# DuckTapeDevOps/kubernetes-cloud

Measured on AMD Instinct MI355X. Metric: GPT-J-6B finetune tokens/sec, higher is better.
Workload: dtype bf16; 1 GPU; model=gpt-j-6b, global_batch=32, micro_batch=16, grad_accum=2, seq_len=2048, parallelism=dp1, activation_checkpointing=False

## Files before the change

csrc/kernels/attention.hip:

```cpp
#include "common.h"

#define LOG2E 1.4426950408889634f
#define LN2 0.6931471805599453f

struct AttnParams {
  const bf16_t* q; const bf16_t* k; const bf16_t* v;
  bf16_t* o; float* lse;
  long long q_sb, q_st, q_sh, k_sb, k_st, k_sh, v_sb, v_st, v_sh;
  long long o_sb, o_st, o_sh;
  int B, Sq, Sk, H, Hkv, d_real, causal;
  float scale;
  const float* alibi;
  const int* kv_len;
  const int* fix_flags;
  int window;
  const unsigned* key_mask;
  int km_words;
};

struct AttnBwdParams {
  const bf16_t* q; const bf16_t* k; const bf16_t* v; const bf16_t* o;
  const bf16_t* dout; bf16_t* dq; bf16_t* dk; bf16_t* dv;
  const float* lse; const float* delta;
  long long q_sb, q_st, q_sh, k_sb, k_st, k_sh, v_sb, v_st, v_sh;
// ... 822 lines not shown
                                    long long do_sh, int B, int S, int H,
                                    int d_real, hipStream_t stream) {
  int nc = (d_real + 7) / 8;
  int tpr = 1;
  while (tpr < nc && tpr < 64) tpr <<= 1;
  const int rpb = 256 / tpr;
  const long long rows = (long long)B * H * S;
  const long long grid = (rows + rpb - 1) / rpb;
  hipLaunchKernelGGL(attn_bwd_preprocess_kernel, dim3((unsigned)grid), dim3(256), 0, stream,
                     (const bf16_t*)o, (const bf16_t*)dout, delta, o_sb, o_st, o_sh,
                     do_sb, do_st, do_sh, B, S, H, d_real, tpr);
  return 0;
}

KCA_API int kca_attn_bwd_tiled(const void* q, const void* k, const void* v, const void* dout,
                               void* dq, void* dk, void* dv, const float* lse, const float* delta,
                               long long q_sb, long long q_st, long long q_sh, long long k_sb,
                               long long k_st, long long k_sh, long long v_sb, long long v_st,
                               long long v_sh, long long do_sb, long long do_st, long long do_sh,
                               long long dq_sb, long long dq_st, long long dq_sh, long long dk_sb,
                               long long dk_st, long long dk_sh, long long dv_sb, long long dv_st,
                               long long dv_sh, int B, int Sq, int Sk, int H, int Hkv, int d,
                               int causal, float scale, hipStream_t stream);

KCA_API int kca_attn_bwd(const void* q, const void* k, const void* v,
                         const void* o, const void* dout, void* dq, void* dk,
                         void* dv, const float* lse, const float* delta,
                         long long q_sb, long long q_st, long long q_sh,
                         long long k_sb, long long k_st, long long k_sh,
                         long long v_sb, long long v_st, long long v_sh,
                         long long do_sb, long long do_st, long long do_sh,
                         long long dq_sb, long long dq_st, long long dq_sh,
                         long long dk_sb, long long dk_st, long long dk_sh,
                         long long dv_sb, long long dv_st, long long dv_sh,
                         int B, int Sq, int Sk, int H, int Hkv, int d_real,
                         int causal, float scale, const float* alibi,
                         const int* kv_len, int window, const unsigned* key_mask, hipStream_t stream) {
  if (d_real % 8 || H % Hkv || window < 0) return 1;
  if (g_attn_tiled && !alibi && !kv_len && !window && !key_mask &&
      kca_attn_bwd_tiled(q, k, v, dout, dq, dk, dv, lse, delta, q_sb, q_st, q_sh, k_sb, k_st, k_sh,
                         v_sb, v_st, v_sh, do_sb, do_st, do_sh, dq_sb, dq_st, dq_sh, dk_sb, dk_st,
                         dk_sh, dv_sb, dv_st, dv_sh, B, Sq, Sk, H, Hkv, d_real, causal, scale,
                         stream) == 0)
    return 0;
  const int D = pick_d(d_real);
  AttnBwdParams p{(const bf16_t*)q, (const bf16_t*)k, (const bf16_t*)v, (const bf16_t*)o,
                  (const bf16_t*)dout, (bf16_t*)dq, (bf16_t*)dk, (bf16_t*)dv, lse, delta,
                  q_sb, q_st, q_sh, k_sb, k_st, k_sh, v_sb, v_st, v_sh,
                  do_sb, do_st, do_sh, dq_sb, dq_st, dq_sh, dk_sb, dk_st, dk_sh,
                  dv_sb, dv_st, dv_sh,
                  B, Sq, Sk, H, Hkv, d_real, causal, scale, alibi, kv_len, window, key_mask, (Sk + 31) / 32};
  if (D == 256) {
    dim3 h2(((Sq + 127) / 128) * B * H);
    dim3 g1w(((Sk + 63) / 64) * B * Hkv);
    if (causal) {
      hipLaunchKernelGGL((attn_bwd_dkdv_kernel<256, true>), g1w, dim3(256), 0, stream, p);
      hipLaunchKernelGGL((attn_bwd_dq32_kernel<256, true>), h2, dim3(256), 0, stream, p);
    } else {
      hipLaunchKernelGGL((attn_bwd_dkdv_kernel<256, false>), g1w, dim3(256), 0, stream, p);
      hipLaunchKernelGGL((attn_bwd_dq32_kernel<256, false>), h2, dim3(256), 0, stream, p);
    }
    return 0;
  }
  dim3 g1(((Sk + 63) / 64) * B * Hkv);
  dim3 g2(((Sq + 63) / 64) * B * H);
  ATTN_D_DISPATCH(D, {
    if (causal) {
      hipLaunchKernelGGL((attn_bwd_dkdv_kernel<DD, true>), g1, dim3(256), 0, stream, p);
      hipLaunchKernelGGL((attn_bwd_dq_kernel<DD, true>), g2, dim3(256), 0, stream, p);
    } else {
      hipLaunchKernelGGL((attn_bwd_dkdv_kernel<DD, false>), g1, dim3(256), 0, stream, p);
      hipLaunchKernelGGL((attn_bwd_dq_kernel<DD, false>), g2, dim3(256), 0, stream, p);
    }
  });
  return 0;
}
```

csrc/kernels/attention_tiled.hip:

```cpp
#include "common.h"

#include <type_traits>

namespace {

constexpr float kLog2e = 1.4426950408889634f;
constexpr float kLn2 = 0.6931471805599453f;
constexpr float kRescaleThr = 8.0f;

#ifdef KCA_ATTN_STAMPS
__device__ unsigned long long g_attn_stamps[64];
__device__ __forceinline__ unsigned long long ast_now() {
  unsigned long long t;
  __builtin_amdgcn_sched_barrier(0);
  asm volatile("s_memtime %0\n\ts_waitcnt lgkmcnt(0)" : "=s"(t)::"memory");
  __builtin_amdgcn_sched_barrier(0);
  return t;
}
#define ASTAMP_DECL                                            \
  unsigned long long st_acc_[8] = {0, 0, 0, 0, 0, 0, 0, 0}; \
  unsigned long long st_prev_ = ast_now();
#define ASTAMP(k)                           \
  do {                                      \
    const unsigned long long n_ = ast_now(); \
// ... 669 lines not shown
    const int lid128 = bh * nqb128 + (CAUSAL ? nqb128 - 1 - qb128 : qb128);
    if (lane == 0) p.flags[lid128 * 4 + w128] = any_bad;
  }
  const float inv = ltot > 0.f ? 1.f / ltot : 0.f;
  if (hh == 0 && p.lse)
    p.lse[((long long)b * p.H + h) * p.Sq + qrow] = ltot > 0.f ? (m + log2f(ltot)) * kLn2 : INFINITY;
  asm volatile("s_waitcnt vmcnt(0) lgkmcnt(0)" ::: "memory");
  __syncthreads();
  store_tile_lds<D, D>(p.o + b * p.o_sb + h * p.o_sh + (long long)q0 * p.o_st, p.o_st, oacc, lane, inv,
                       smem + wave * 32 * D * 2);
  ASTAMP(6);
  ASTAMP_FLUSH(48);
}

struct FastBwdParams {
  const bf16_t* q; const bf16_t* k; const bf16_t* v; const bf16_t* dout;
  bf16_t* dq; bf16_t* dk; bf16_t* dv;
  const float* lse; const float* delta;
  long long q_sb, q_st, q_sh, k_sb, k_st, k_sh, v_sb, v_st, v_sh, do_sb, do_st, do_sh;
  long long dq_sb, dq_st, dq_sh, dk_sb, dk_st, dk_sh, dv_sb, dv_st, dv_sh;
  int B, Sq, Sk, H, Hkv;
  float scale;
};

template <int D>
__device__ __forceinline__ void row_bases(int l32, int hh, int& e, int& o) {
  const int xr = (l32 >> 2) & 3;
  e = (l32 >> 3) * 16 * D + 64 * (l32 & 7) + 16 * (hh ^ xr);
  o = (l32 >> 3) * 16 * D + 64 * (l32 & 7) + 16 * ((2 + hh) ^ xr);
}
template <int D>
__device__ __forceinline__ void tr_bases(int lane, int& b1, int& b2) {
  const int hh = lane >> 5, gi = lane & 15;
  const int c3 = 2 * ((lane >> 4) & 1) + ((gi & 3) >> 1);
  b1 = 64 * (4 * hh + (gi >> 2)) + 16 * (c3 ^ hh) + 8 * (gi & 1);
  b2 = 16 * D + 64 * (4 * hh + (gi >> 2)) + 16 * (c3 ^ hh ^ 2) + 8 * (gi & 1);
}
template <int D>
__device__ __forceinline__ bf16x8 tr_frag(const char* img, int b1, int b2, int s, int db) {
  return cat8(lds_tr4(img, b1 + 2 * s * 16 * D + 512 * db), lds_tr4(img, b2 + 2 * s * 16 * D + 512 * db));
}
template <int D>
__device__ __forceinline__ bf16x8 row_frag(const char* img, int be, int bo, int s) {
  return lds_b128(img, ((s & 1) ? bo : be) + 512 * (s >> 1));
}

// ... 130 lines not shown
        if (db + 1 < D / 32) {
          t0[(db + 1) & 1] = tr_frag<D>(Ks, b1, b2, 0, db + 1);
          t1[(db + 1) & 1] = tr_frag<D>(Ks, b1, b2, 1, db + 1);
          __builtin_amdgcn_sched_group_barrier(0x100, 4, 0);
        }
        dq[db] = __builtin_amdgcn_mfma_f32_32x32x16_bf16(t0[db & 1], d0, dq[db], 0, 0, 0);
        dq[db] = __builtin_amdgcn_mfma_f32_32x32x16_bf16(t1[db & 1], d1, dq[db], 0, 0, 0);
        __builtin_amdgcn_sched_group_barrier(0x8, 2, 0);
      }
    }
    ASTAMP(4);
    asm volatile("" ::: "memory");
    if (t + 1 < ntiles) stg.store(sk, sv, smem + ((t + 1) & 1) * 2 * TILE);
    __syncthreads();
    ASTAMP(5);
  };
  const int nfree = CAUSAL ? ntiles - 4 : ntiles;
  for (int t = 0; t < nfree; ++t) tile_step(t, std::false_type{});
  for (int t = max(nfree, 0); t < ntiles; ++t) tile_step(t, std::true_type{});
  store_tile_lds<D, DS>(p.dq + b * p.dq_sb + h * p.dq_sh + (long long)q0 * p.dq_st, p.dq_st, dq, lane, p.scale,
                        smem + wave * 32 * D * 2);
  ASTAMP(6);
  ASTAMP_FLUSH(16);
}

template <int D, bool CAUSAL, int DS = D>
__global__ void __launch_bounds__(256, (D <= 64 && !CAUSAL) ? 3 : 1) attn_bwd_dkdv_tiled_kernel(FastBwdParams p) {
  constexpr int BK = 128, BQ = 32;
  constexpr int TILE = BQ * D * 2;
  using Stg = StagerFor<D, DS>;
  constexpr int NCH = D / 8, NCS = DS / 8, CPT = Stg::CPT;
  constexpr int KSD = DS / 16;
  constexpr int VOFF = 4 * TILE;
  constexpr int LOFF = VOFF + 4 * TILE;
  __shared__ __attribute__((aligned(16))) char smem[LOFF + 2 * 64 * 4];
  ASTAMP_DECL

  const int tid = threadIdx.x, lane = tid & 63, wave = tid >> 6;
  const int l32 = lane & 31, hh = lane >> 5;
  const int nkb = p.Sk / BK;
  const int lid = xcd_remap(blockIdx.x, gridDim.x);
  const int kb = lid % nkb, bh = lid / nkb;
  const int b = bh / p.Hkv, hk = bh % p.Hkv;
  const int grp = p.H / p.Hkv;
  const int off = p.Sk - p.Sq;
  const int kw = kb * BK + wave * 32;
// ... 149 lines not shown
    }
    ASTAMP(4);
    asm volatile("" ::: "memory");
    if (it + 1 < total) KCA_DKDV_STORE((it + 1) & 1);
    __syncthreads();
    ASTAMP(5);
  };
  for (int it = 0; it < total; ++it) tile_step(it, std::integral_constant<bool, CAUSAL>{});
#undef KCA_DKDV_LOAD
#undef KCA_DKDV_STORE
  if constexpr (D == 96) {
    store_acc_t<D>(p.dk + b * p.dk_sb + hk * p.dk_sh + (long long)key * p.dk_st, dk, hh, p.scale);
    store_acc_t<D>(p.dv + b * p.dv_sb + hk * p.dv_sh + (long long)key * p.dv_st, dv, hh, 1.f);
  } else {
    store_tile_lds<D, DS>(p.dk + b * p.dk_sb + hk * p.dk_sh + (long long)kw * p.dk_st, p.dk_st, dk, lane, p.scale,
                      smem + wave * 32 * D * 2);
    store_tile_lds<D, DS>(p.dv + b * p.dv_sb + hk * p.dv_sh + (long long)kw * p.dv_st, p.dv_st, dv, lane, 1.f,
                      smem + wave * 32 * D * 2);
  }
  ASTAMP(6);
  ASTAMP_FLUSH(32);
}

template <int D, bool CAUSAL>
__global__ void __launch_bounds__(512, 1) attn_bwd_dkdv_w8_kernel(FastBwdParams p) {
  constexpr int BK = 128, BQ = 32;
  constexpr int TILE = BQ * D * 2;
  using Stg = Stager<D, true, 512>;
  constexpr int CPT = Stg::CPT, KSD = D / 16;
  constexpr int PSZ = 4 * 64 * 16;
  constexpr int POFF = 3 * 2 * TILE;
  constexpr int LOFF = POFF + 2 * 4 * PSZ;
  __shared__ __attribute__((aligned(16))) char smem[LOFF + 3 * 64 * 4];
  static_assert(8 * 32 * D * 2 <= LOFF, "epilogue images of the 8 waves");
  ASTAMP_DECL

  const int tid = threadIdx.x, lane = tid & 63;
  const int wave = __builtin_amdgcn_readfirstlane(tid >> 6);
  const int pw = wave & 3;
  const bool kside = wave < 4;
  const int l32 = lane & 31, hh = lane >> 5;
  const int nkb = p.Sk / BK;
  const int lid = xcd_remap(blockIdx.x, gridDim.x);
  const int kb = lid % nkb, bh = lid / nkb;
  const int b = bh / p.H, h = bh % p.H;
  const int off = p.Sk - p.Sq;
  const int kw = kb * BK + pw * 32;
  const int key = kw + l32;
// ... 105 lines not shown
        for (int i = 0; i < D / 16; ++i) {
          if (i + 2 < D / 16) {
            f[(i + 2) % 3] = tr_frag<D>(Gs, b1, b2, i & 1, (i + 2) >> 1);
            __builtin_amdgcn_sched_group_barrier(0x100, 2, 0);
          }
          acc[i >> 1] = __builtin_amdgcn_mfma_f32_32x32x16_bf16(f[i % 3], (i & 1) ? p1 : p0, acc[i >> 1], 0, 0, 0);
          __builtin_amdgcn_sched_group_barrier(0x8, 1, 0);
        }
      }
      ASTAMP(4);
      asm volatile("" ::: "memory");
      if (t + 1 < total) store_tile(nxt);
      __syncthreads();
      ASTAMP(5);
    };
    int cur = 0;
    for (int t = 0; t < total; ++t) {
      const int nxt = cur == 2 ? 0 : cur + 1;
      v_step(t, cur, nxt);
      cur = nxt;
    }
    __syncthreads();
  } else {
    auto k_step = [&](int t, int cur, int nxt) {
      const char* Qs = smem + cur * 2 * TILE;
      const char* Gs = Qs + TILE;
      const float* ls = reinterpret_cast<const float*>(smem + LOFF) + cur * 64 + 32;
      const float* pb = reinterpret_cast<const float*>(smem + POFF + ((t & 1) * 4 + pw) * PSZ);
      ASTAMP(1);
      f32x16 dpacc;
#pragma unroll
      for (int r = 0; r < 16; ++r) dpacc[r] = 0.f;
      {
        constexpr int PF = 1;
        bf16x8 f[PF + 1];
#pragma unroll
        for (int s = 0; s < PF; ++s) f[s] = row_frag<D>(Gs, be, bo, s);
        __builtin_amdgcn_sched_group_barrier(0x100, PF, 0);
#pragma unroll
        for (int s = 0; s < KSD; ++s) {
          if (s + PF < KSD) {
            f[(s + PF) % (PF + 1)] = row_frag<D>(Gs, be, bo, s + PF);
            __builtin_amdgcn_sched_group_barrier(0x100, 1, 0);
          }
          dpacc = __builtin_amdgcn_mfma_f32_32x32x16_bf16(f[s % (PF + 1)], rf[s], dpacc, 0, 0, 0);
          __builtin_amdgcn_sched_group_barrier(0x8, 1, 0);
        }
      }
      ASTAMP(2);
      load_tile(min(t + 2, total - 1));
      asm volatile("" ::: "memory");
      bf16x8 s0, s1;
#pragma unroll
      for (int g = 0; g < 4; ++g) {
        const f32x4 pg = *reinterpret_cast<const f32x4*>(pb + (g * 64 + lane) * 4);
        const f32x4 dq4 = *reinterpret_cast<const f32x4*>(ls + 8 * g + 4 * hh);
#pragma unroll
        for (int j = 0; j < 4; ++j) {
          const int r = 4 * g + j;
          const float ds = pg[j] * (dpacc[r] - dq4[j]);
          if (r < 8) s0[r] = (__bf16)ds;
          else s1[r - 8] = (__bf16)ds;
        }
      }
      ASTAMP(3);
      {
        bf16x8 f[3];
        f[0] = tr_frag<D>(Qs, b1, b2, 0, 0);
        f[1] = tr_frag<D>(Qs, b1, b2, 1, 0);
        __builtin_amdgcn_sched_group_barrier(0x100, 4, 0);
#pragma unroll
        for (int i = 0; i < D / 16; ++i) {
          if (i + 2 < D / 16) {
            f[(i + 2) % 3] = tr_frag<D>(Qs, b1, b2, i & 1, (i + 2) >> 1);
            __builtin_amdgcn_sched_group_barrier(0x100, 2, 0);
          }
          acc[i >> 1] = __builtin_amdgcn_mfma_f32_32x32x16_bf16(f[i % 3], (i & 1) ? s1 : s0, acc[i >> 1], 0, 0, 0);
          __builtin_amdgcn_sched_group_barrier(0x8, 1, 0);
        }
      }
      ASTAMP(4);
      asm volatile("" ::: "memory");
      if (t + 2 < total) store_tile(nxt);
      __syncthreads();
      ASTAMP(5);
    };
    if (total > 1) {
// ... 6 lines not shown
      const int nxt = cur == 0 ? 2 : cur - 1;
      k_step(t, cur, nxt);
      cur = cur == 2 ? 0 : cur + 1;
    }
  }
  __builtin_amdgcn_s_setprio(0);
  {
    bf16_t* dst = kside ? p.dk + b * p.dk_sb + h * p.dk_sh + (long long)kw * p.dk_st
                        : p.dv + b * p.dv_sb + h * p.dv_sh + (long long)kw * p.dv_st;
    store_tile_lds<D>(dst, kside ? p.dk_st : p.dv_st, acc, lane, kside ? p.scale : 1.f, smem + wave * 32 * D * 2);
  }
  ASTAMP(6);
  if (!kside) {
    ASTAMP_FLUSH(40);
  } else {
    ASTAMP_FLUSH(56);
  }
}

inline bool offsets_fit(long long rows, long long stride) { return (rows + 128) * stride * 2 < (1ll << 31); }

}

static int g_attn_variant = 3;
KCA_API int kca_attn_set_variant(int v) {
  g_attn_variant = v;
  return 0;
}

KCA_API int kca_attn_fwd_tiled(const void* q, const void* k, const void* v, void* o, float* lse,
                               long long q_sb, long long q_st, long long q_sh, long long k_sb,
                               long long k_st, long long k_sh, long long v_sb, long long v_st,
                               long long v_sh, long long o_sb, long long o_st, long long o_sh,
                               int B, int Sq, int Sk, int H, int Hkv, int d, int causal,
                               float scale, int rowsum_col, int max_col, int* flags, hipStream_t stream) {
  if ((d != 48 && d != 64 && d != 96 && d != 128 && d != 160 && d != 256) || Sq % 128 || Sk % 32 || Sq <= 0 ||
      H % Hkv || !flags)
    return 1;
  if (max_col >= 0 && (max_col != 40 || rowsum_col != 40 || d != 48)) return 1;
  if (d == 48 && causal) return 1;
  if (rowsum_col >= 0 && (rowsum_col != 40 || (d != 64 && d != 48) || causal)) return 1;
  if (causal && Sk < Sq) return 1;
  if (!offsets_fit(Sk, k_st) || !offsets_fit(Sk, v_st)) return 1;
  FastFwdParams p{(const bf16_t*)q, (const bf16_t*)k, (const bf16_t*)v, (bf16_t*)o, lse, flags,
                  q_sb, q_st, q_sh, k_sb, k_st, k_sh, v_sb, v_st, v_sh, o_sb, o_st, o_sh,
                  B, Sq, Sk, H, Hkv, scale};
  dim3 grid((Sq / 128) * B * H);
// ... 93 lines not shown
      hipLaunchKernelGGL((attn_bwd_dkdv_tiled_kernel<96, false>), g1, dim3(256), 0, stream, p);
      hipLaunchKernelGGL((attn_bwd_dq_tiled_kernel<96, false>), g2, dim3(256), 0, stream, p);
    }
  } else if (d == 128) {
    if (causal) {
      hipLaunchKernelGGL((attn_bwd_dkdv_tiled_kernel<128, true>), g1, dim3(256), 0, stream, p);
      hipLaunchKernelGGL((attn_bwd_dq_tiled_kernel<128, true>), g2, dim3(256), 0, stream, p);
    } else {
      hipLaunchKernelGGL((attn_bwd_dkdv_tiled_kernel<128, false>), g1, dim3(256), 0, stream, p);
      hipLaunchKernelGGL((attn_bwd_dq_tiled_kernel<128, false>), g2, dim3(256), 0, stream, p);
    }
  } else {
    if (causal) {
      hipLaunchKernelGGL((attn_bwd_dkdv_tiled_kernel<64, true>), g1, dim3(256), 0, stream, p);
      hipLaunchKernelGGL((attn_bwd_dq_tiled_kernel<64, true>), g2, dim3(256), 0, stream, p);
    } else {
      hipLaunchKernelGGL((attn_bwd_dkdv_tiled_kernel<64, false>), g1, dim3(256), 0, stream, p);
      hipLaunchKernelGGL((attn_bwd_dq_tiled_kernel<64, false>), g2, dim3(256), 0, stream, p);
    }
  }
  return 0;
}

#ifdef KCA_ATTN_STAMPS
KCA_API int kca_attn_stamps(unsigned long long* host, int reset) {
  if (hipMemcpyFromSymbol(host, HIP_SYMBOL(g_attn_stamps), sizeof(unsigned long long) * 64) != hipSuccess) return 1;
  if (reset) {
    unsigned long long z[64] = {0};
    if (hipMemcpyToSymbol(HIP_SYMBOL(g_attn_stamps), z, sizeof(z)) != hipSuccess) return 1;
  }
  return 0;
}
#endif
```

kubernetes_cloud_amd/ops/_lib.py:

```python
from __future__ import annotations

import ctypes
import os
import threading

import torch

_HERE = os.path.dirname(os.path.abspath(__file__))
LIB_DIR = os.path.join(os.path.dirname(_HERE), "_lib")
DEBUG = os.environ.get("KCA_DEBUG", "0") in ("1", "true")
KERNEL_LIB = os.path.join(LIB_DIR, "libkca_kernels_debug.so" if DEBUG else "libkca_kernels.so")
KERNEL_LIB = os.environ.get("KCA_KERNEL_LIB") or KERNEL_LIB
ATTN_VARIANT_ENV = os.environ.get("KCA_ATTN_VARIANT")

_lock = threading.Lock()
_lib = None
_err: str | None = None

P = ctypes.c_void_p
I = ctypes.c_int
LL = ctypes.c_longlong
F = ctypes.c_float

_SIGS = {
# ... 7 lines not shown
    "kca_gelu_bwd": [P, P, P, LL, I, P],
    "kca_quick_gelu_fwd": [P, P, LL, P],
    "kca_quick_gelu_bwd": [P, P, P, LL, P],
    "kca_geglu_fwd": [P, P, LL, I, P],
    "kca_add_bias_nhwc": [P, P, P, P, LL, I, P],
    "kca_add_bias2_nhwc": [P, P, P, P, P, LL, I, P],
    "kca_colsum_bf16": [P, P, I, I, I, P],
    "kca_geglu_bwd": [P, P, P, LL, I, P],
    "kca_rope": [P, P, I, I, LL, I, LL, LL, LL, LL, I, I, P, P, P, F, P],
    "kca_accum_grad": [P, P, F, I, LL, P],
    "kca_accum_grad_pair": [P, P, P, F, LL, P],
    "kca_accum_grad_multi": [P, I, F, P],
    "kca_cast_f32_bf16": [P, P, LL, P],
    "kca_ema": [P, P, F, LL, P],
    "kca_cross_entropy_fwd": [P, LL, P, I, I, I, P, P, P],
    "kca_cross_entropy_bwd": [P, LL, P, P, P, F, I, I, I, P, LL, P],
    "kca_adamw": [P, P, P, P, P, LL, P, F, F, F, F, F, F, F, P, P, P],
    "kca_sumsq": [P, LL, P, P, P],
    "kca_adamw8bit": [P, P, P, P, P, P, P, LL, P, F, F, F, F, F, F, F, P, P, P],
    "kca_clip_coef": [P, F, F, P, P, P, P],
    "kca_attn_fwd": [P] * 5 + [LL] * 12 + [I] * 7 + [F, P, P, I, P, I, I, P, P],
    "kca_attn_bwd_preprocess": [P, P, P, LL, LL, LL, LL, LL, LL, I, I, I, I, P],
    "kca_attn_bwd": [P] * 10 + [LL] * 21 + [I] * 7 + [F, P, P, I, P, P],
    "kca_attn_fwd_wide": [P] * 5 + [LL] * 12 + [I] * 6 + [F, P, P],
    "kca_attn_set_tiled": [I],
    "kca_attn_set_variant": [I],
    "kca_transpose_bf16": [P, LL, P, LL, I, I, P],
    "kca_gelu_fwd_t": [P, LL, P, LL, P, LL, I, I, I, P],
    "kca_gelu_bwd_t": [P, LL, P, LL, P, LL, P, LL, P, I, I, I, P],
    "kca_transpose_colsum": [P, LL, P, LL, P, I, I, P],
    "kca_col_reduce_f32": [P, I, I, P, P, P],
    "kca_accum_grad_2d": [P, P, LL, I, I, F, I, P],
    "kca_groupnorm_fwd": [P, P, P, P, P, P, P, I, I, I, I, F, I, P],
    "kca_groupnorm_bwd": [P, P, P, P, P, P, P, P, P, P, I, I, I, I, I, P],
    "kca_groupnorm_nhwc_ws": [I, I, I],
    "kca_groupnorm_nhwc_fwd": [P, P, P, P, P, P, P, I, I, I, I, F, I, P],
    "kca_groupnorm_nhwc_fwd_add": [P, P, P, P, LL, P, P, P, P, I, I, I, I, F, I, P],
    "kca_groupnorm_nhwc_cat_fwd": [P, P, P, P, P, P, P, P, P, P, I, I, I, I, I, I, F, I, P],
    "kca_groupnorm_nhwc_bwd": [P, P, P, P, P, P, P, P, P, P, I, I, I, I, I, P],
    "kca_skinny_set_smallk": [I],
    "kca_conv3x3_fwd": [P, P, P, P, I, I, I, I, I, P],
    "kca_conv3x3_set_variant": [I],
    "kca_conv3x3_wflip": [P, P, I, I, P],
    "kca_conv3x3_wgrad_splits": [I, I, I, I, I],
    "kca_conv3x3_wgrad": [P, P, P, P, I, I, I, I, I, I, P],
    "kca_skinny_gemm": [P, LL, P, P, P, LL, I, I, I, I, P],
# ... 3 lines not shown
    "kca_ln_rows": [P, LL, P, P, P, LL, P, P, F, P, I, I, P],
    "kca_embed_ln_rows": [P, LL, P, P, P, I, P, LL, P, P, F, P, I, I, P],
    "kca_decode_prep": [P, LL, I, I, I, I, I, I, P, P, P, P, P, P, LL, LL, LL, P, I, I, P],
    "kca_decode_chunk": [I, I, I],
    "kca_decode_set_stamps": [P],
    "kca_decode_attn": [P, LL, P, P, LL, LL, LL, P, P, P, LL, P, LL, I, I, I, I, I, I, F, P, P, I, I, I, P],
    "kca_sd_noise_prep": [P, P, P, P, P, P, P, P, P, I, I, I, I, F, I, ctypes.c_ulonglong, LL, I, P],
    "kca_mse_split_fwd": [P, P, LL, LL, F, P, I, P, P],
    "kca_mse_split_bwd": [P, P, P, LL, LL, F, P, P],
    "kca_sd_lms_step": [P, P, P, P, LL, P, I, I, I, I, I, F, F, F, P],
    "kca_decode_prep_attn": [P, LL, P, P, LL, LL, LL, P, P, P, LL, P, LL, I, I, I, I, I, I, F, P, P, I, I, I, I, P,
                             P, I, I, P],
    "kca_im2col2x2_nhwc": [P, P, I, I, I, I, P],
    "kca_phase_to_dense_nhwc": [P, P, P, I, I, I, I, P],
    "kca_upsample2x_nhwc": [P, P, I, I, I, I, P],
    "kca_dense_to_phase_nhwc": [P, P, I, I, I, I, P],
    "kca_col2im2x2_nhwc": [P, P, I, I, I, I, P],
    "kca_pad_br_nhwc": [P, P, I, I, I, I, P],
    "kca_gemv_dual_ln": [P, P, I, P, P, I, P, P, P, P, P, P, P, F, P, P, P, P, I, P],
    "kca_sample_logits": [P, LL, I, I, I, P, P, P, P, P, P, P, I, P, LL, P, P, P, P, P, I, P],
}


_SIGS["kca_decode_prep_attn_gemv"] = _SIGS["kca_decode_prep_attn"][:-2] + [P, P, P, P, I, I, I, I, P]

for _n in ("kca_decode_prep_attn", "kca_ln_rows", "kca_embed_ln_rows", "kca_decode_prep_attn_gemv",
           "kca_gemv_dual_ln", "kca_skinny_gemm"):
    _SIGS[_n + "_f16"] = _SIGS[_n]


def _load():
    global _lib, _err
    if _lib is not None or _err is not None:
        return _lib
    with _lock:
        if _lib is not None or _err is not None:
            return _lib
        if not os.path.exists(KERNEL_LIB):
            _err = f"{KERNEL_LIB} not built (run `python tools/build_ext.py`)"
            return None
        try:
            lib = ctypes.CDLL(KERNEL_LIB, mode=ctypes.RTLD_GLOBAL)
        except OSError as e:
            _err = f"failed to load {KERNEL_LIB}: {e}"
            return None
        for name, argtypes in _SIGS.items():
            fn = getattr(lib, name, None)
            if fn is None:
                continue
            fn.argtypes = argtypes
            fn.restype = ctypes.c_int
        if ATTN_VARIANT_ENV is not None and hasattr(lib, "kca_attn_set_variant"):
            lib.kca_attn_set_variant(int(ATTN_VARIANT_ENV))
        _lib = lib
        return _lib


def available() -> bool:
    return _load() is not None


def require():
    lib = _load()
    if lib is None:
        raise RuntimeError(
            "kubernetes_cloud_amd native kernels unavailable: " + str(_err)
            + " -- refusing to fall back to eager PyTorch on a GPU tensor")
    return lib


def has(name: str) -> bool:
    lib = _load()
    return lib is not None and hasattr(lib, name)

# ... 57 lines not shown
```

kubernetes_cloud_amd/ops/attention.py:

```python
from __future__ import annotations

import math

import torch

from . import _lib
from .rope import apply_rotary_


def attention_reference(q, k, v, causal: bool, scale: float | None = None,
                        kv_len: torch.Tensor | None = None, alibi: torch.Tensor | None = None,
                        window: int = 0):
    B, Sq, H, D = q.shape
    Sk, Hkv = k.shape[1], k.shape[2]
    scale = scale if scale is not None else 1.0 / math.sqrt(D)
    qf = q.float().transpose(1, 2)
    kf = k.float().transpose(1, 2)
    vf = v.float().transpose(1, 2)
    if Hkv != H:
        rep = H // Hkv
        kf = kf.repeat_interleave(rep, dim=1)
        vf = vf.repeat_interleave(rep, dim=1)
    s = torch.matmul(qf, kf.transpose(-1, -2)) * scale
    qi = torch.arange(Sq, device=q.device)[:, None]
# ... 2 lines not shown
    if alibi is not None:
        s = s + alibi.float().view(1, H, 1, 1) * (ki - qi - off).float()
    mask = torch.zeros(B, 1, Sq, Sk, dtype=torch.bool, device=q.device)
    if causal:
        mask = mask | (ki > qi + off)
    if window:
        mask = mask | (ki <= qi + off - window)
    if kv_len is not None and kv_len.dtype == torch.bool:
        mask = mask | ~kv_len.to(q.device).view(B, 1, 1, Sk)
    elif kv_len is not None:
        mask = mask | (ki[None, None] >= kv_len.view(B, 1, 1, 1).to(q.device))
    s = s.masked_fill(mask, float("-inf"))
    lse = torch.logsumexp(s, dim=-1)
    p = torch.exp(s - lse[..., None])
    p = torch.nan_to_num(p, nan=0.0)
    o = torch.matmul(p, vf).transpose(1, 2)
    return o.to(q.dtype), lse


def set_tiled_path(enable: bool) -> None:
    _lib.call("kca_attn_set_tiled", int(bool(enable)))


DEFAULT_VARIANT = 3
_VARIANT = [int(_lib.ATTN_VARIANT_ENV) if _lib.ATTN_VARIANT_ENV is not None else DEFAULT_VARIANT]


def set_variant(v: int) -> int:
    _lib.call("kca_attn_set_variant", int(v))
    old, _VARIANT[0] = _VARIANT[0], int(v)
    return old


def _strides(t):
    return t.stride(0), t.stride(1), t.stride(2)


def pack_key_mask(mask: torch.Tensor) -> torch.Tensor:
    B, Sk = mask.shape
    W = (Sk + 31) // 32
    m = torch.zeros(B, W * 32, dtype=torch.int64, device=mask.device)
    m[:, :Sk] = mask.to(torch.int64)
    words = (m.view(B, W, 32) << torch.arange(32, device=mask.device, dtype=torch.int64)).sum(-1)
    words = torch.where(words >= 2 ** 31, words - 2 ** 32, words)
    return words.to(torch.int32).contiguous()


def _masks(kv_len):
    if kv_len is None:
        return None, None
    return (kv_len, None) if kv_len.dim() == 1 else (None, kv_len)


def _fwd(q, k, v, causal, scale, kv_len, alibi, out=None, window: int = 0, rowsum_col: int = -1,
         max_col: int = -1, lse=None, flags=None):
    B, Sq, H, D = q.shape
    Sk, Hkv = k.shape[1], k.shape[2]
    o = out if out is not None else torch.empty(B, Sq, H, D, device=q.device, dtype=q.dtype)
    if lse is None:
        lse = torch.empty(B, H, Sq, device=q.device, dtype=torch.float32)
    if flags is None:
        flags = torch.empty(4 * ((Sq + 127) // 128) * B * H, device=q.device, dtype=torch.int32)
    lens, km = _masks(kv_len)
    _lib.call("kca_attn_fwd", q.data_ptr(), k.data_ptr(), v.data_ptr(), o.data_ptr(), lse.data_ptr(),
              *_strides(q), *_strides(k), *_strides(v), *_strides(o),
              B, Sq, Sk, H, Hkv, D, int(causal), float(scale), _lib.ptr(alibi), _lib.ptr(lens),
              int(window), _lib.ptr(km), int(rowsum_col), int(max_col), flags.data_ptr(), _lib.stream())
    return o, lse


def _bwd(q, k, v, o, do, lse, dq, dk, dv, causal, scale, kv_len, alibi, window: int = 0):
    B, Sq, H, D = q.shape
    Sk, Hkv = k.shape[1], k.shape[2]
    delta = torch.empty(B, H, Sq, device=q.device, dtype=torch.float32)
    _lib.call("kca_attn_bwd_preprocess", o.data_ptr(), do.data_ptr(), delta.data_ptr(),
              *_strides(o), *_strides(do), B, Sq, H, D, _lib.stream())
    _lib.call("kca_attn_bwd", q.data_ptr(), k.data_ptr(), v.data_ptr(), o.data_ptr(), do.data_ptr(),
              dq.data_ptr(), dk.data_ptr(), dv.data_ptr(), lse.data_ptr(), delta.data_ptr(),
              *_strides(q), *_strides(k), *_strides(v), *_strides(do),
              *_strides(dq), *_strides(dk), *_strides(dv),
              B, Sq, Sk, H, Hkv, D, int(causal), float(scale), _lib.ptr(alibi), _lib.ptr(_masks(kv_len)[0]),
              int(window), _lib.ptr(_masks(kv_len)[1]), _lib.stream())


def _check(q, k, v):
    for t in (q, k, v):
        if t.dim() != 4 or t.stride(-1) != 1:
            raise ValueError("attention expects [B, S, H, D] views with unit last stride")
        if t.dtype != torch.bfloat16:
            raise ValueError("native attention is bf16")
    D = q.shape[-1]
    if D % 8 or D > 256:
        raise ValueError(f"head_dim {D} unsupported (multiple of 8, <= 256)")


class _FlashAttnFn(torch.autograd.Function):
    @staticmethod
    def forward(ctx, q, k, v, causal, scale, kv_len, alibi, window):
        _check(q, k, v)
        o, lse = _fwd(q, k, v, causal, scale, kv_len, alibi, window=window)
        ctx.save_for_backward(q, k, v, o, lse, kv_len, alibi)
        ctx.causal, ctx.scale, ctx.window = causal, scale, window
        return o

    @staticmethod
    def backward(ctx, do):
        q, k, v, o, lse, kv_len, alibi = ctx.saved_tensors
        do = do.contiguous()
        dq = torch.empty(q.shape, device=q.device, dtype=q.dtype)
        dk = torch.empty(k.shape, device=k.device, dtype=k.dtype)
        dv = torch.empty(v.shape, device=v.device, dtype=v.dtype)
        _bwd(q, k, v, o, do, lse, dq, dk, dv, ctx.causal, ctx.scale, kv_len, alibi, ctx.window)
        return dq, dk, dv, None, None, None, None, None


def native_mask(kv_len, device):
    if kv_len is None:
        return None
    if kv_len.dtype == torch.bool:
        return pack_key_mask(kv_len.to(device))
    return kv_len.to(device=device, dtype=torch.int32).contiguous()


def flash_attention(q: torch.Tensor, k: torch.Tensor, v: torch.Tensor, causal: bool = False,
                    scale: float | None = None, kv_len: torch.Tensor | None = None,
                    alibi: torch.Tensor | None = None, window: int = 0, rowsum_col: int = -1,
                    max_col: int = -1) -> torch.Tensor:
    scale = scale if scale is not None else 1.0 / math.sqrt(q.shape[-1])
    if alibi is not None:
        alibi = alibi.to(device=q.device, dtype=torch.float32).contiguous()
    if rowsum_col >= 0 and _lib.use_native(q, k, v) and not torch.is_grad_enabled():
        _check(q, k, v)
        return _fwd(q, k, v, causal, scale, native_mask(kv_len, q.device), alibi, window=window,
                    rowsum_col=rowsum_col, max_col=max_col)[0]
    if max_col >= 0:
# ... 29 lines not shown
    @staticmethod
    def forward(ctx, qkv, H, D, rot, interleaved, base, causal, scale, kv_len):
        B, S, _ = qkv.shape
        v5 = qkv.view(B, S, 3, H, D)
        q, k, v = v5[:, :, 0], v5[:, :, 1], v5[:, :, 2]
        if rot > 0:
            apply_rotary_(q, k, rot, S, interleaved, base, 1.0)
        o, lse = _fwd(q, k, v, causal, scale, kv_len, None)
        ctx.save_for_backward(qkv, o, lse, kv_len)
        ctx.cfg = (H, D, rot, interleaved, base, causal, scale)
        return o.view(B, S, H * D)

    @staticmethod
    def backward(ctx, do):
        qkv, o, lse, kv_len = ctx.saved_tensors
        H, D, rot, interleaved, base, causal, scale = ctx.cfg
        B, S, _ = qkv.shape
        v5 = qkv.view(B, S, 3, H, D)
        q, k, v = v5[:, :, 0], v5[:, :, 1], v5[:, :, 2]
        dqkv = torch.empty_like(qkv)
        d5 = dqkv.view(B, S, 3, H, D)
        dq, dk, dv = d5[:, :, 0], d5[:, :, 1], d5[:, :, 2]
        do = do.contiguous().view(B, S, H, D)
        _bwd(q, k, v, o, do, lse, dq, dk, dv, causal, scale, kv_len, None)
        if rot > 0:
            apply_rotary_(dq, dk, rot, S, interleaved, base, -1.0)
        return dqkv, None, None, None, None, None, None, None, None


def qkv_rope_attention(qkv: torch.Tensor, n_heads: int, head_dim: int, rot: int,
                       interleaved: bool, causal: bool = True, base: float = 10000.0,
                       scale: float | None = None,
                       kv_len: torch.Tensor | None = None) -> torch.Tensor:
    B, S, _ = qkv.shape
    scale = scale if scale is not None else 1.0 / math.sqrt(head_dim)
    if _lib.use_native(qkv):
        return _QKVRopeAttnFn.apply(qkv.contiguous(), n_heads, head_dim, rot, interleaved, base,
                                    causal, scale, native_mask(kv_len, qkv.device))
    v5 = qkv.view(B, S, 3, n_heads, head_dim)
    q, k, v = v5[:, :, 0], v5[:, :, 1], v5[:, :, 2]
    if rot > 0:
        q, k = _rope_out_of_place(q, k, rot, interleaved, base)
    o, _ = attention_reference(q, k, v, causal, scale, kv_len, None)
    return o.reshape(B, S, n_heads * head_dim)


def _rope_out_of_place(q, k, rot, interleaved, base):
# ... 9 lines not shown
```

kubernetes_cloud_amd/ops/fused_block.py:

```python
from __future__ import annotations

import torch
import torch.nn.functional as F

from . import _lib, grad_sink
from .attention import _bwd as _attn_bwd
from .attention import _fwd as _attn_fwd
from .attention import native_mask
from .linear import transpose
from .rope import apply_rotary_


def eligible(cfg) -> bool:
    d, f = cfg.hidden, cfg.ffn_dim
    return (cfg.parallel_residual and cfg.shared_ln and cfg.rotary_dim > 0 and not cfg.qkv_bias
            and not cfg.out_bias and not cfg.alibi and not cfg.attention_layers
            and d % 64 == 0 and f % 64 == 0 and cfg.head_dim in (64, 128, 256))


class FusedParallelBlock:

    def __init__(self, blk):
        self.blk = blk
        self.tanh = blk.mlp.approx == "tanh"

    def refresh(self):
        pass

    def applies(self, x: torch.Tensor, kv_len=None) -> bool:
        a, m = self.blk.attn, self.blk.mlp
# ... 72 lines not shown
        st = _lib.stream()
        dm2 = dm.reshape(T, d).contiguous() if dm is not None else torch.zeros(T, d, device=dev, dtype=dt)
        da2 = da.reshape(T, d).contiguous() if da is not None else torch.zeros(T, d, device=dev, dtype=dt)

        dmt = torch.empty(d, T, device=dev, dtype=dt)
        part = torch.empty(T // 64, d, device=dev, dtype=torch.float32) if b_needed(mlp.fc_out) else None
        _lib.call("kca_transpose_colsum", dm2.data_ptr(), d, dmt.data_ptr(), T, _lib.ptr(part), T, d, st)
        g_b_out = _emit(mlp.fc_out.bias, _col_sums(part, dt)) if part is not None else None
        dg = F.linear(dm2, mlp.fc_out.weight_t)
        g_fc_out = _emit_wgrad(mlp.fc_out.weight, dmt, gt)
        if da2.data_ptr() != dm2.data_ptr():
            dat = transpose(da2)
        else:
            dat = dmt
        g_out = _emit_wgrad(a.out.weight, dat, transpose(o))
        do = F.linear(da2, a.out.weight_t).view(B, S, H, D)
        del dat, dmt

        q5 = qkv.view(B, S, 3, H, D)
        dqkv = torch.empty_like(qkv)
        d5 = dqkv.view(B, S, 3, H, D)
        dq, dk, dv = d5[:, :, 0], d5[:, :, 1], d5[:, :, 2]
        _attn_bwd(q5[:, :, 0], q5[:, :, 1], q5[:, :, 2], o.view(B, S, H, D), do, lse, dq, dk, dv, True,
                  a.scale, kv_len, None)
        apply_rotary_(dq, dk, cfg.rotary_dim, S, cfg.rotary_interleaved, cfg.rotary_base, -1.0)
        del do

        du = torch.empty_like(u)
        dut = torch.empty(f, T, device=dev, dtype=dt)
        part = torch.empty(T // 64, f, device=dev, dtype=torch.float32) if b_needed(mlp.fc_in) else None
        _lib.call("kca_gelu_bwd_t", dg.data_ptr(), f, u.data_ptr(), f, du.data_ptr(), f, dut.data_ptr(), T,
                  _lib.ptr(part), T, f, int(fb.tanh), st)
        del dg
        g_b_in = _emit(mlp.fc_in.bias, _col_sums(part, dt)) if part is not None else None

        dx = None
        if ctx.needs_input_grad[0]:
            dx = F.linear(dqkv, a.qkv.weight_t)
            dx.addmm_(du, mlp.fc_in.weight_t.t())
        xt = transpose(x.reshape(T, d))
        g_fc_in = _emit_wgrad(mlp.fc_in.weight, dut, xt)
        del dut, du
        g_qkv = _emit_wgrad(a.qkv.weight, transpose(dqkv), xt)
        return (dx.view(B, S, d) if dx is not None else None, g_qkv, g_out, g_fc_in, g_b_in, g_fc_out, g_b_out,
                None, None)


# ... 6 lines not shown
```

Baseline: 34810 tokens/s.

## Store attention dS in a workspace and compute dQ from it without recompute

The dK/dV backward kernel now also writes the bf16 dS tile for every query/key block into a per-head workspace of size B*H*Sq*Sk. A new dQ kernel then streams K and dS from that workspace and accumulates dQ = dS·K, instead of recomputing QK^T, the softmax and dP in a separate dQ pass. This is the new default (variant 7) for head dim 256 with equal Q and KV heads, and the Python layers allocate the workspace per backward call. The cost is a large extra HBM write and read per layer (about 2 GiB at this batch and sequence length) and a transient memory allocation, traded against the matmul and exp work saved in the dQ pass.

```diff
diff --git a/csrc/kernels/attention.hip b/csrc/kernels/attention.hip
--- a/csrc/kernels/attention.hip
+++ b/csrc/kernels/attention.hip
@@ -868,8 +868,17 @@
                                long long dk_st, long long dk_sh, long long dv_sb, long long dv_st,
                                long long dv_sh, int B, int Sq, int Sk, int H, int Hkv, int d,
                                int causal, float scale, hipStream_t stream);
-
-KCA_API int kca_attn_bwd(const void* q, const void* k, const void* v,
+KCA_API int kca_attn_bwd_tiled_ws(const void* q, const void* k, const void* v, const void* dout,
+                                  void* dq, void* dk, void* dv, const float* lse, const float* delta,
+                                  long long q_sb, long long q_st, long long q_sh, long long k_sb,
+                                  long long k_st, long long k_sh, long long v_sb, long long v_st,
+                                  long long v_sh, long long do_sb, long long do_st, long long do_sh,
+                                  long long dq_sb, long long dq_st, long long dq_sh, long long dk_sb,
+                                  long long dk_st, long long dk_sh, long long dv_sb, long long dv_st,
+                                  long long dv_sh, int B, int Sq, int Sk, int H, int Hkv, int d,
+                                  int causal, float scale, void* ws, long long ws_bytes, hipStream_t stream);
+
+KCA_API int kca_attn_bwd_ws(const void* q, const void* k, const void* v,
                          const void* o, const void* dout, void* dq, void* dk,
                          void* dv, const float* lse, const float* delta,
                          long long q_sb, long long q_st, long long q_sh,
@@ -881,13 +890,14 @@
                          long long dv_sb, long long dv_st, long long dv_sh,
                          int B, int Sq, int Sk, int H, int Hkv, int d_real,
                          int causal, float scale, const float* alibi,
-                         const int* kv_len, int window, const unsigned* key_mask, hipStream_t stream) {
+                         const int* kv_len, int window, const unsigned* key_mask, void* ws,
+                         long long ws_bytes, hipStream_t stream) {
   if (d_real % 8 || H % Hkv || window < 0) return 1;
   if (g_attn_tiled && !alibi && !kv_len && !window && !key_mask &&
-      kca_attn_bwd_tiled(q, k, v, dout, dq, dk, dv, lse, delta, q_sb, q_st, q_sh, k_sb, k_st, k_sh,
-                         v_sb, v_st, v_sh, do_sb, do_st, do_sh, dq_sb, dq_st, dq_sh, dk_sb, dk_st,
-                         dk_sh, dv_sb, dv_st, dv_sh, B, Sq, Sk, H, Hkv, d_real, causal, scale,
-                         stream) == 0)
+      kca_attn_bwd_tiled_ws(q, k, v, dout, dq, dk, dv, lse, delta, q_sb, q_st, q_sh, k_sb, k_st, k_sh,
+                            v_sb, v_st, v_sh, do_sb, do_st, do_sh, dq_sb, dq_st, dq_sh, dk_sb, dk_st,
+                            dk_sh, dv_sb, dv_st, dv_sh, B, Sq, Sk, H, Hkv, d_real, causal, scale, ws,
+                            ws_bytes, stream) == 0)
     return 0;
   const int D = pick_d(d_real);
   AttnBwdParams p{(const bf16_t*)q, (const bf16_t*)k, (const bf16_t*)v, (const bf16_t*)o,
@@ -921,3 +931,22 @@
   });
   return 0;
 }
+
+KCA_API int kca_attn_bwd(const void* q, const void* k, const void* v,
+                         const void* o, const void* dout, void* dq, void* dk,
+                         void* dv, const float* lse, const float* delta,
+                         long long q_sb, long long q_st, long long q_sh,
+                         long long k_sb, long long k_st, long long k_sh,
+                         long long v_sb, long long v_st, long long v_sh,
+                         long long do_sb, long long do_st, long long do_sh,
+                         long long dq_sb, long long dq_st, long long dq_sh,
+                         long long dk_sb, long long dk_st, long long dk_sh,
+                         long long dv_sb, long long dv_st, long long dv_sh,
+                         int B, int Sq, int Sk, int H, int Hkv, int d_real,
+                         int causal, float scale, const float* alibi,
+                         const int* kv_len, int window, const unsigned* key_mask, hipStream_t stream) {
+  return kca_attn_bwd_ws(q, k, v, o, dout, dq, dk, dv, lse, delta, q_sb, q_st, q_sh, k_sb, k_st, k_sh, v_sb, v_st,
+                         v_sh, do_sb, do_st, do_sh, dq_sb, dq_st, dq_sh, dk_sb, dk_st, dk_sh, dv_sb, dv_st, dv_sh,
+                         B, Sq, Sk, H, Hkv, d_real, causal, scale, alibi, kv_len, window, key_mask, nullptr, 0,
+                         stream);
+}
diff --git a/csrc/kernels/attention_tiled.hip b/csrc/kernels/attention_tiled.hip
--- a/csrc/kernels/attention_tiled.hip
+++ b/csrc/kernels/attention_tiled.hip
@@ -715,6 +715,9 @@
   int B, Sq, Sk, H, Hkv;
   float scale;
 };
+struct FastBwdWsParams : FastBwdParams {
+  bf16_t* ws;
+};
 
 template <int D>
 __device__ __forceinline__ void row_bases(int l32, int hh, int& e, int& o) {
@@ -891,6 +894,131 @@
                         smem + wave * 32 * D * 2);
   ASTAMP(6);
   ASTAMP_FLUSH(16);
+}
+
+template <int D, bool CAUSAL>
+__global__ void __launch_bounds__(256, 2) attn_bwd_dq_ds_kernel(FastBwdWsParams p) {
+  constexpr int BM = 128, BN = 32;
+  constexpr int TILE = BN * D * 2;
+  constexpr int NCH = D / 8, CPT = 32 * NCH / 256, RPI = 256 / NCH;
+  constexpr int DST = BN * 32 * 2;
+  constexpr int DOFF = 2 * TILE;
+  __shared__ __attribute__((aligned(16))) char smem[4 * TILE];
+  static_assert(DOFF + 2 * 4 * DST <= 4 * TILE && 256 % NCH == 0, "dQ from dS: LDS plan");
+
+  const int tid = threadIdx.x, lane = tid & 63, wave = tid >> 6;
+  const int hh = lane >> 5;
+  const int nqb = p.Sq / BM;
+  const int lid = xcd_remap(blockIdx.x, gridDim.x);
+  const int qi = lid % nqb;
+  const int qb = CAUSAL ? (nqb - 1 - qi) : qi;
+  const int bh = lid / nqb;
+  const int b = bh / p.H, h = bh % p.H;
+  const int off = p.Sk - p.Sq;
+  const int q0 = qb * BM + wave * 32;
+  int kv_hi = p.Sk;
+  if (CAUSAL) kv_hi = min(kv_hi, qb * BM + BM + off);
+  const int ntiles = (kv_hi + BN - 1) / BN;
+
+  f32x16 dq[D / 32];
+#pragma unroll
+  for (int i = 0; i < D / 32; ++i)
+#pragma unroll
+    for (int r = 0; r < 16; ++r) dq[i][r] = 0.f;
+
+  const __amdgpu_buffer_rsrc_t rk = head_rsrc(p.k + b * p.k_sb + h * p.k_sh);
+  int vok[CPT], lk[CPT];
+#pragma unroll
+  for (int i = 0; i < CPT; ++i) {
+    vok[i] = (int)(((long long)(tid / NCH + i * RPI) * p.k_st + (tid % NCH) * 8) * 2);
+    lk[i] = img_off<D>(tid / NCH + i * RPI, tid % NCH);
+  }
+  const __amdgpu_buffer_rsrc_t rw = head_rsrc(p.ws + (long long)bh * p.Sq * p.Sk);
+  const int ws_row = __builtin_amdgcn_readfirstlane((q0 / 32) * (p.Sk / 32) * DST);
+  const int wv = lane * 16;
+  char* const dsl = smem + DOFF + wave * DST;
+  int dsw[4], dsr[4];
+#pragma unroll
+  for (int n = 0; n < 4; ++n) {
+    const int l32 = lane & 31, key = 8 * n + 4 * hh + ((lane & 15) >> 2), qq = 4 * ((lane >> 4) & 1) + (lane & 3);
+    dsw[n] = 64 * l32 + 8 * ((hh + 2 * n) ^ (l32 >> 2));
+    dsr[n] = 64 * key + 8 * (qq ^ (key >> 2));
+  }
+  int b1, b2;
+  tr_bases<D>(lane, b1, b2);
+
+  constexpr int PD = 2;
+  u32x4 sk[CPT], sd[PD][2];
+  auto load_k = [&](int t) {
+    const int sok = __builtin_amdgcn_readfirstlane((int)(t * BN * p.k_st * 2));
+#pragma unroll
+    for (int i = 0; i < CPT; ++i) {
+      const auto a = __builtin_amdgcn_raw_buffer_load_b128(rk, vok[i], sok, 0);
+      sk[i] = *reinterpret_cast<const u32x4*>(&a);
+    }
+  };
+  auto load_ds = [&](int t, auto set) {
+    const int so = __builtin_amdgcn_readfirstlane(ws_row + t * DST);
+#pragma unroll
+    for (int i = 0; i < 2; ++i) {
+      const auto a = __builtin_amdgcn_raw_buffer_load_b128(rw, wv, so + i * (DST / 2), 2);
+      sd[decltype(set)::value][i] = *reinterpret_cast<const u32x4*>(&a);
+    }
+  };
+  auto store_tile = [&](int buf, auto set) {
+    constexpr int J = decltype(set)::value;
+#pragma unroll
+    for (int i = 0; i < CPT; ++i) *reinterpret_cast<u32x4*>(smem + buf * TILE + lk[i]) = sk[i];
+#pragma unroll
+    for (int i = 0; i < 2; ++i) {
+      *reinterpret_cast<u32x2*>(dsl + buf * 4 * DST + dsw[2 * i]) = u32x2{sd[J][i][0], sd[J][i][1]};
+      *reinterpret_cast<u32x2*>(dsl + buf * 4 * DST + dsw[2 * i + 1]) = u32x2{sd[J][i][2], sd[J][i][3]};
+    }
+  };
+  const int last = ntiles - 1;
+
+  load_k(0);
+  load_ds(0, std::integral_constant<int, 0>{});
+  store_tile(0, std::integral_constant<int, 0>{});
+  static_for<1, PD>([&](auto T) { load_ds(min(decltype(T)::value, last), T); });
+  __builtin_amdgcn_sched_barrier(0);
+  load_k(min(1, last));
+  __builtin_amdgcn_sched_barrier(0);
+  load_ds(min(PD, last), std::integral_constant<int, 0>{});
+  __syncthreads();
+  auto tile_step = [&](int t, auto jc) {
+    constexpr int NX = (decltype(jc)::value + 1) % PD;
+    const char* Ks = smem + (t & 1) * TILE;
+    const char* ds = dsl + (t & 1) * 4 * DST;
+    const bf16x8 d0 = cat8(lds_tr4(ds, dsr[0]), lds_tr4(ds, dsr[1]));
+    const bf16x8 d1 = cat8(lds_tr4(ds, dsr[2]), lds_tr4(ds, dsr[3]));
+    {
+      bf16x8 t0[2], t1[2];
+      t0[0] = tr_frag<D>(Ks, b1, b2, 0, 0);
+      t1[0] = tr_frag<D>(Ks, b1, b2, 1, 0);
+      __builtin_amdgcn_sched_group_barrier(0x100, 8, 0);
+#pragma unroll
+      for (int db = 0; db < D / 32; ++db) {
+        if (db + 1 < D / 32) {
+          t0[(db + 1) & 1] = tr_frag<D>(Ks, b1, b2, 0, db + 1);
+          t1[(db + 1) & 1] = tr_frag<D>(Ks, b1, b2, 1, db + 1);
+          __builtin_amdgcn_sched_group_barrier(0x100, 4, 0);
+        }
+        dq[db] = __builtin_amdgcn_mfma_f32_32x32x16_bf16(t0[db & 1], d0, dq[db], 0, 0, 0);
+        dq[db] = __builtin_amdgcn_mfma_f32_32x32x16_bf16(t1[db & 1], d1, dq[db], 0, 0, 0);
+        __builtin_amdgcn_sched_group_barrier(0x8, 2, 0);
+      }
+    }
+    asm volatile("" ::: "memory");
+    if (t + 1 < ntiles) store_tile((t + 1) & 1, std::integral_constant<int, NX>{});
+    load_k(min(t + 2, last));
+    load_ds(min(t + 1 + PD, last), std::integral_constant<int, NX>{});
+    __syncthreads();
+  };
+  for (int t = 0; t < ntiles; t += PD)
+    static_for<0, PD>([&](auto J) { tile_step(t + decltype(J)::value, J); });
+  store_tile_lds<D>(p.dq + b * p.dq_sb + h * p.dq_sh + (long long)q0 * p.dq_st, p.dq_st, dq, lane, p.scale,
+                    smem + wave * 32 * D * 2);
 }
 
 template <int D, bool CAUSAL, int DS = D>
@@ -1086,8 +1214,31 @@
   ASTAMP_FLUSH(32);
 }
 
-template <int D, bool CAUSAL>
-__global__ void __launch_bounds__(512, 1) attn_bwd_dkdv_w8_kernel(FastBwdParams p) {
+template <bool ON>
+struct DsEmitter {
+  __device__ __forceinline__ void init(const FastBwdParams&, int, int, int, int) {}
+  __device__ __forceinline__ void store(const bf16x8&, const bf16x8&, int) const {}
+};
+template <>
+struct DsEmitter<true> {
+  __amdgpu_buffer_rsrc_t r_;
+  int v_, dt_, t0_;
+  __device__ __forceinline__ void init(const FastBwdWsParams& p, int bh, int lane, int q_lo, int kw) {
+    r_ = head_rsrc(p.ws + (long long)bh * p.Sq * p.Sk);
+    v_ = lane * 16;
+    dt_ = (p.Sk / 32) * 2048;
+    t0_ = (q_lo / 32) * dt_ + (kw / 32) * 2048;
+  }
+  __device__ __forceinline__ void store(const bf16x8& s0, const bf16x8& s1, int t) const {
+    const int so = __builtin_amdgcn_readfirstlane(t0_ + t * dt_);
+    __builtin_amdgcn_raw_buffer_store_b128(*reinterpret_cast<const u32x4*>(&s0), r_, v_, so, 2);
+    __builtin_amdgcn_raw_buffer_store_b128(*reinterpret_cast<const u32x4*>(&s1), r_, v_, so + 1024, 2);
+  }
+};
+
+template <int D, bool CAUSAL, bool EMIT_DS = false>
+__global__ void __launch_bounds__(512, 1)
+    attn_bwd_dkdv_w8_kernel(std::conditional_t<EMIT_DS, FastBwdWsParams, FastBwdParams> p) {
   constexpr int BK = 128, BQ = 32;
   constexpr int TILE = BQ * D * 2;
   using Stg = Stager<D, true, 512>;
@@ -1239,6 +1390,8 @@
     }
     __syncthreads();
   } else {
+    DsEmitter<EMIT_DS> emit;
+    emit.init(p, bh, lane, q_lo, kw);
     auto k_step = [&](int t, int cur, int nxt) {
       const char* Qs = smem + cur * 2 * TILE;
       const char* Gs = Qs + TILE;
@@ -1280,6 +1433,7 @@
           else s1[r - 8] = (__bf16)ds;
         }
       }
+      emit.store(s0, s1, t);
       ASTAMP(3);
       {
         bf16x8 f[3];
@@ -1332,7 +1486,7 @@
 
 }
 
-static int g_attn_variant = 3;
+static int g_attn_variant = 7;
 KCA_API int kca_attn_set_variant(int v) {
   g_attn_variant = v;
   return 0;
@@ -1472,6 +1626,44 @@
   return 0;
 }
 
+KCA_API long long kca_attn_bwd_ws_bytes(int B, int Sq, int Sk, int H, int Hkv, int d, int causal) {
+  if (d != 256 || H != Hkv || B <= 0 || H <= 0 || Sq <= 0 || Sq % 128 || Sk % 128 || (causal && Sk < Sq)) return 0;
+  if ((long long)Sq * Sk * 2 >= (1ll << 31)) return 0;
+  return (long long)B * H * Sq * Sk * 2;
+}
+
+KCA_API int kca_attn_bwd_tiled_ws(const void* q, const void* k, const void* v, const void* dout,
+                                  void* dq, void* dk, void* dv, const float* lse, const float* delta,
+                                  long long q_sb, long long q_st, long long q_sh, long long k_sb,
+                                  long long k_st, long long k_sh, long long v_sb, long long v_st,
+                                  long long v_sh, long long do_sb, long long do_st, long long do_sh,
+                                  long long dq_sb, long long dq_st, long long dq_sh, long long dk_sb,
+                                  long long dk_st, long long dk_sh, long long dv_sb, long long dv_st,
+                                  long long dv_sh, int B, int Sq, int Sk, int H, int Hkv, int d,
+                                  int causal, float scale, void* ws, long long ws_bytes, hipStream_t stream) {
+  const long long need = kca_attn_bwd_ws_bytes(B, Sq, Sk, H, Hkv, d, causal);
+  if ((g_attn_variant & 6) != 6 || !ws || need == 0 || ws_bytes < need || !offsets_fit(Sk, k_st) ||
+      !offsets_fit(Sk, v_st) || !offsets_fit(Sq, q_st) || !offsets_fit(Sq, do_st))
+    return kca_attn_bwd_tiled(q, k, v, dout, dq, dk, dv, lse, delta, q_sb, q_st, q_sh, k_sb, k_st, k_sh, v_sb,
+                              v_st, v_sh, do_sb, do_st, do_sh, dq_sb, dq_st, dq_sh, dk_sb, dk_st, dk_sh, dv_sb,
+                              dv_st, dv_sh, B, Sq, Sk, H, Hkv, d, causal, scale, stream);
+  FastBwdWsParams p{{(const bf16_t*)q, (const bf16_t*)k, (const bf16_t*)v, (const bf16_t*)dout,
+                     (bf16_t*)dq, (bf16_t*)dk, (bf16_t*)dv, lse, delta,
+                     q_sb, q_st, q_sh, k_sb, k_st, k_sh, v_sb, v_st, v_sh, do_sb, do_st, do_sh,
+                     dq_sb, dq_st, dq_sh, dk_sb, dk_st, dk_sh, dv_sb, dv_st, dv_sh,
+                     B, Sq, Sk, H, Hkv, scale},
+                    (bf16_t*)ws};
+  dim3 g1((Sk / 128) * B * H), g2((Sq / 128) * B * H);
+  if (causal) {
+    hipLaunchKernelGGL((attn_bwd_dkdv_w8_kernel<256, true, true>), g1, dim3(512), 0, stream, p);
+    hipLaunchKernelGGL((attn_bwd_dq_ds_kernel<256, true>), g2, dim3(256), 0, stream, p);
+  } else {
+    hipLaunchKernelGGL((attn_bwd_dkdv_w8_kernel<256, false, true>), g1, dim3(512), 0, stream, p);
+    hipLaunchKernelGGL((attn_bwd_dq_ds_kernel<256, false>), g2, dim3(256), 0, stream, p);
+  }
+  return 0;
+}
+
 #ifdef KCA_ATTN_STAMPS
 KCA_API int kca_attn_stamps(unsigned long long* host, int reset) {
   if (hipMemcpyFromSymbol(host, HIP_SYMBOL(g_attn_stamps), sizeof(unsigned long long) * 64) != hipSuccess) return 1;
diff --git a/kubernetes_cloud_amd/ops/_lib.py b/kubernetes_cloud_amd/ops/_lib.py
--- a/kubernetes_cloud_amd/ops/_lib.py
+++ b/kubernetes_cloud_amd/ops/_lib.py
@@ -53,6 +53,8 @@
     "kca_attn_fwd": [P] * 5 + [LL] * 12 + [I] * 7 + [F, P, P, I, P, I, I, P, P],
     "kca_attn_bwd_preprocess": [P, P, P, LL, LL, LL, LL, LL, LL, I, I, I, I, P],
     "kca_attn_bwd": [P] * 10 + [LL] * 21 + [I] * 7 + [F, P, P, I, P, P],
+    "kca_attn_bwd_ws": [P] * 10 + [LL] * 21 + [I] * 7 + [F, P, P, I, P, P, LL, P],
+    "kca_attn_bwd_ws_bytes": [I] * 7,
     "kca_attn_fwd_wide": [P] * 5 + [LL] * 12 + [I] * 6 + [F, P, P],
     "kca_attn_set_tiled": [I],
     "kca_attn_set_variant": [I],
@@ -102,6 +104,8 @@
 }
 
 
+_RESTYPES = {"kca_attn_bwd_ws_bytes": ctypes.c_longlong}
+
 _SIGS["kca_decode_prep_attn_gemv"] = _SIGS["kca_decode_prep_attn"][:-2] + [P, P, P, P, I, I, I, I, P]
 
 for _n in ("kca_decode_prep_attn", "kca_ln_rows", "kca_embed_ln_rows", "kca_decode_prep_attn_gemv",
@@ -129,7 +133,7 @@
             if fn is None:
                 continue
             fn.argtypes = argtypes
-            fn.restype = ctypes.c_int
+            fn.restype = _RESTYPES.get(name, ctypes.c_int)
         if ATTN_VARIANT_ENV is not None and hasattr(lib, "kca_attn_set_variant"):
             lib.kca_attn_set_variant(int(ATTN_VARIANT_ENV))
         _lib = lib
diff --git a/kubernetes_cloud_amd/ops/attention.py b/kubernetes_cloud_amd/ops/attention.py
--- a/kubernetes_cloud_amd/ops/attention.py
+++ b/kubernetes_cloud_amd/ops/attention.py
@@ -48,7 +48,7 @@
     _lib.call("kca_attn_set_tiled", int(bool(enable)))
 
 
-DEFAULT_VARIANT = 3
+DEFAULT_VARIANT = 7
 _VARIANT = [int(_lib.ATTN_VARIANT_ENV) if _lib.ATTN_VARIANT_ENV is not None else DEFAULT_VARIANT]
 
 
@@ -95,18 +95,30 @@
     return o, lse
 
 
-def _bwd(q, k, v, o, do, lse, dq, dk, dv, causal, scale, kv_len, alibi, window: int = 0):
+def bwd_workspace(q, k, causal):
+    if not _VARIANT[0] & 4:
+        return None
+    B, Sq, H, D = q.shape
+    n = _lib.require().kca_attn_bwd_ws_bytes(B, Sq, k.shape[1], H, k.shape[2], D, int(causal))
+    return torch.empty(n, device=q.device, dtype=torch.uint8) if n > 0 else None
+
+
+def _bwd(q, k, v, o, do, lse, dq, dk, dv, causal, scale, kv_len, alibi, window: int = 0, ws=None):
     B, Sq, H, D = q.shape
     Sk, Hkv = k.shape[1], k.shape[2]
     delta = torch.empty(B, H, Sq, device=q.device, dtype=torch.float32)
     _lib.call("kca_attn_bwd_preprocess", o.data_ptr(), do.data_ptr(), delta.data_ptr(),
               *_strides(o), *_strides(do), B, Sq, H, D, _lib.stream())
-    _lib.call("kca_attn_bwd", q.data_ptr(), k.data_ptr(), v.data_ptr(), o.data_ptr(), do.data_ptr(),
-              dq.data_ptr(), dk.data_ptr(), dv.data_ptr(), lse.data_ptr(), delta.data_ptr(),
-              *_strides(q), *_strides(k), *_strides(v), *_strides(do),
-              *_strides(dq), *_strides(dk), *_strides(dv),
-              B, Sq, Sk, H, Hkv, D, int(causal), float(scale), _lib.ptr(alibi), _lib.ptr(_masks(kv_len)[0]),
-              int(window), _lib.ptr(_masks(kv_len)[1]), _lib.stream())
+    args = (q.data_ptr(), k.data_ptr(), v.data_ptr(), o.data_ptr(), do.data_ptr(),
+            dq.data_ptr(), dk.data_ptr(), dv.data_ptr(), lse.data_ptr(), delta.data_ptr(),
+            *_strides(q), *_strides(k), *_strides(v), *_strides(do),
+            *_strides(dq), *_strides(dk), *_strides(dv),
+            B, Sq, Sk, H, Hkv, D, int(causal), float(scale), _lib.ptr(alibi), _lib.ptr(_masks(kv_len)[0]),
+            int(window), _lib.ptr(_masks(kv_len)[1]))
+    if ws is None:
+        _lib.call("kca_attn_bwd", *args, _lib.stream())
+    else:
+        _lib.call("kca_attn_bwd_ws", *args, ws.data_ptr(), ws.numel() * ws.element_size(), _lib.stream())
 
 
 def _check(q, k, v):
@@ -136,7 +148,8 @@
         dq = torch.empty(q.shape, device=q.device, dtype=q.dtype)
         dk = torch.empty(k.shape, device=k.device, dtype=k.dtype)
         dv = torch.empty(v.shape, device=v.device, dtype=v.dtype)
-        _bwd(q, k, v, o, do, lse, dq, dk, dv, ctx.causal, ctx.scale, kv_len, alibi, ctx.window)
+        _bwd(q, k, v, o, do, lse, dq, dk, dv, ctx.causal, ctx.scale, kv_len, alibi, ctx.window,
+             ws=bwd_workspace(q, k, ctx.causal))
         return dq, dk, dv, None, None, None, None, None
 
 
@@ -212,7 +225,7 @@
         d5 = dqkv.view(B, S, 3, H, D)
         dq, dk, dv = d5[:, :, 0], d5[:, :, 1], d5[:, :, 2]
         do = do.contiguous().view(B, S, H, D)
-        _bwd(q, k, v, o, do, lse, dq, dk, dv, causal, scale, kv_len, None)
+        _bwd(q, k, v, o, do, lse, dq, dk, dv, causal, scale, kv_len, None, ws=bwd_workspace(q, k, causal))
         if rot > 0:
             apply_rotary_(dq, dk, rot, S, interleaved, base, -1.0)
         return dqkv, None, None, None, None, None, None, None, None
diff --git a/kubernetes_cloud_amd/ops/fused_block.py b/kubernetes_cloud_amd/ops/fused_block.py
--- a/kubernetes_cloud_amd/ops/fused_block.py
+++ b/kubernetes_cloud_amd/ops/fused_block.py
@@ -6,6 +6,7 @@
 from . import _lib, grad_sink
 from .attention import _bwd as _attn_bwd
 from .attention import _fwd as _attn_fwd
+from .attention import bwd_workspace as _attn_bwd_workspace
 from .attention import native_mask
 from .linear import transpose
 from .rope import apply_rotary_
@@ -124,7 +125,7 @@
         d5 = dqkv.view(B, S, 3, H, D)
         dq, dk, dv = d5[:, :, 0], d5[:, :, 1], d5[:, :, 2]
         _attn_bwd(q5[:, :, 0], q5[:, :, 1], q5[:, :, 2], o.view(B, S, H, D), do, lse, dq, dk, dv, True,
-                  a.scale, kv_len, None)
+                  a.scale, kv_len, None, ws=_attn_bwd_workspace(q5[:, :, 0], q5[:, :, 1], True))
         apply_rotary_(dq, dk, cfg.rotary_dim, S, cfg.rotary_interleaved, cfg.rotary_base, -1.0)
         del do
 
```

Measured after the change: 35590 tokens/s, median of 6. 2.2% higher.
